# sanonone/kektordb

Measured on AMD Instinct MI355X. Metric: QPS at recall@10>=0.95, 1Mx768 cosine k=10, higher is better.
Workload: dtype f32

## Files before the change

### kektordb_amd/csrc/kdb_search_core.cuh

```cuda
#pragma once
#include "kdb_device.cuh"
#include <math.h>

#ifndef KDB_F32_ROWS2
#define KDB_F32_ROWS2 4
#endif
#ifndef KDB_F32_ROWS6
#define KDB_F32_ROWS6 2
#endif
#ifndef KDB_F32_ROWS
#define KDB_F32_ROWS 3
#endif
#ifndef KDB_F32_DUAL
#define KDB_F32_DUAL 1
#endif
#ifndef KDB_WIDE4_ROWS
#define KDB_WIDE4_ROWS 1
#ifndef KDB_LDS_MERGE
#define KDB_LDS_MERGE 1
#endif
#endif
#ifndef KDB_F16_ROWS
#define KDB_F16_ROWS 2
#endif
#ifdef KDB_SEARCH_TIMERS
#define KDB_T(x) x
#else
#define KDB_T(x)
#endif
namespace kdbcore {

struct WaveLds {
    float *q;
    float *beam_d;
    uint32_t *beam_id;
    uint32_t *nb_id;
    float *nb_d;
    uint32_t *marks;
    uint32_t beam_cap;
    float *nr_d;
    uint32_t *nr_id;
    uint32_t nr_cap;
    uint32_t *nb_lo;
    uint32_t *beam_lo;
    uint32_t *nr_lo;
    uint32_t *ctl;
    float *ins_d;
    uint32_t *ins_id;
    uint32_t ins_cap = 0;
    float qn_up = INFINITY;
};
enum { KDB_W_MB_SEQ = 0,
       KDB_W_MB_ARG = 1,
       KDB_W_LEVEL = 2,
       KDB_W_NEXT2 = 3,
       KDB_W_ROWS_SEQ = 4,
       KDB_W_ROWS_N = 5,
       KDB_W_DONE = 6,
       KDB_W_QNORM = 7,
       KDB_W_ALLOW_LO = 8, KDB_W_ALLOW_HI = 9 };
enum { KDB_W_VISIT = 0u, KDB_W_BEGIN = 1u, KDB_W_EXIT = 2u };
constexpr uint32_t KDB_W_N_SKIP = 0xfffffffdu;
constexpr uint32_t KDB_W_N_EXIT = 0xffffffffu;

__device__ __forceinline__ uint32_t uni(uint32_t x) { return (uint32_t)__builtin_amdgcn_readfirstlane((int)x); }
__device__ __forceinline__ float unif(float x) {
    return __builtin_bit_cast(float, __builtin_amdgcn_readfirstlane(__builtin_bit_cast(int, x)));
}
__device__ __forceinline__ float readlane_f(float x, uint32_t l) {
    return __builtin_bit_cast(float, __builtin_amdgcn_readlane(__builtin_bit_cast(int, x), (int)l));
}
__device__ __forceinline__ uint32_t readlane_u(uint32_t x, uint32_t l) {
    return (uint32_t)__builtin_amdgcn_readlane((int)x, (int)l);
}
__device__ __forceinline__ uint32_t shr1_u(uint32_t x) {
    return (uint32_t)__builtin_amdgcn_update_dpp((int)x, (int)x, 0x138, 0xf, 0xf, false);
}
__device__ __forceinline__ float shr1_f(float x) { return __builtin_bit_cast(float, shr1_u(__builtin_bit_cast(uint32_t, x))); }
__device__ __forceinline__ uint32_t shl1_u(uint32_t x) {
    return (uint32_t)__builtin_amdgcn_update_dpp((int)x, (int)x, 0x130, 0xf, 0xf, false);
}
__device__ __forceinline__ float shl1_f(float x) { return __builtin_bit_cast(float, shl1_u(__builtin_bit_cast(uint32_t, x))); }

__device__ __forceinline__ void wave_lds_fence() {
    __builtin_amdgcn_fence(__ATOMIC_ACQ_REL, "wavefront");
    __builtin_amdgcn_wave_barrier();
}

__device__ __forceinline__ float kdb_sane_key(float key) { return key != key ? INFINITY : key; }

__device__ __forceinline__ uint32_t lds_u32_or(const uint32_t *p, uint32_t i, uint32_t n, uint32_t other) {
    const uint32_t x = p[i];
    return i < n ? x : other;
}
__device__ __forceinline__ float lds_f32_or(const float *p, uint32_t i, uint32_t n, float other) {
    const float x = p[i];
    return i < n ? x : other;
}

__device__ __forceinline__ float kdb_query_norm_up(const float *q, uint32_t ld) {
    double sq = 0.0;
    for (uint32_t i = (uint32_t)kdb_lane(); i < ld; i += 64u) {
        const double y = (double)q[i];
        sq += y * y;
    }
#pragma unroll
    for (int o = 32; o >= 1; o >>= 1) sq += __shfl_xor(sq, o, 64);
    const double nrm = sqrt(sq) * (1.0 + 0x1p-20);
    float f = (float)nrm;
    if ((double)f < nrm) f = __uint_as_float(__float_as_uint(f) + 1u);
    return unif(nrm <= 0x1p20 ? f : INFINITY);
}
__device__ __forceinline__ float kdb_perm_f(uint32_t a, uint32_t b, uint32_t sel) { return __uint_as_float(__builtin_amdgcn_perm(a, b, sel)); }
__device__ __forceinline__ float4 kdb_plane_piece(uint32_t wh, uint32_t wh2, uint32_t wl, uint32_t wl2) {
    return make_float4(kdb_perm_f(wh, wl, 0x05040100u), kdb_perm_f(wh, wl, 0x07060302u), kdb_perm_f(wh2, wl2, 0x05040100u), kdb_perm_f(wh2, wl2, 0x07060302u));
}
__device__ __forceinline__ float4 kdb_plane_piece_hi(uint32_t wh, uint32_t wh2) {
    return make_float4(kdb_perm_f(wh, wh, 0x05040c0cu), kdb_perm_f(wh, wh, 0x07060c0cu), kdb_perm_f(wh2, wh2, 0x05040c0cu), kdb_perm_f(wh2, wh2, 0x07060c0cu));
}
template <int NCH, int RR, bool HI>
__device__ __forceinline__ void kdb_planes_partial(const uint4 (&h)[RR][NCH / 2], const uint4 (&l)[RR][NCH / 2], const float4 (&yq)[NCH], float (&p)[RR]) {
    float a[RR][4];
#pragma unroll
    for (int r = 0; r < RR; r++) a[r][0] = a[r][1] = a[r][2] = a[r][3] = 0.f;
#pragma unroll
    for (int i = 0; i < NCH; i++) {
        const float4 y = yq[i];
#pragma unroll
        for (int r = 0; r < RR; r++) {
            const uint4 wh = h[r][i >> 1], wl = l[r][i >> 1];
            const float4 x = HI ? ((i & 1) ? kdb_plane_piece_hi(wh.z, wh.w) : kdb_plane_piece_hi(wh.x, wh.y))
                                : ((i & 1) ? kdb_plane_piece(wh.z, wh.w, wl.z, wl.w) : kdb_plane_piece(wh.x, wh.y, wl.x, wl.y));
            a[r][0] = __builtin_fmaf(y.x, x.x, a[r][0]);
            a[r][1] = __builtin_fmaf(y.y, x.y, a[r][1]);
            a[r][2] = __builtin_fmaf(y.z, x.z, a[r][2]);
            a[r][3] = __builtin_fmaf(y.w, x.w, a[r][3]);
        }
        __builtin_amdgcn_sched_barrier(0);
    }
#pragma unroll
    for (int r = 0; r < RR; r++) p[r] = (a[r][0] + a[r][1]) + (a[r][2] + a[r][3]);
}
template <int NCH, int RR>
__device__ __forceinline__ void kdb_planes_trip(const KdbView &v, const WaveLds &s, uint32_t base, uint32_t n, int g, int t, bool full, float neg_worst) {
    constexpr int NJ = NCH / 2;
    uint32_t rr[RR];
    size_t off[RR];
    uint4 h[RR][NJ], l[RR][NJ];
    float er[RR];
#pragma unroll
    for (int r = 0; r < RR; r++) {
        rr[r] = base + 4u * (uint32_t)r + (uint32_t)g;
        const uint32_t id = lds_u32_or(s.nb_id, rr[r], n, 0u);
        off[r] = (size_t)id * v.ld;
        const uint4 *hp = reinterpret_cast<const uint4 *>(v.walk_hi + off[r]);
#pragma unroll
        for (int j = 0; j < NJ; j++) h[r][j] = hp[t + 16 * j];
        er[r] = full ? v.walk_err[id] : 0.f;
    }
    float4 yq[NCH];
#pragma unroll
    for (int i = 0; i < NCH; i++) yq[i] = reinterpret_cast<const float4 *>(s.q)[t + 16 * i];
    bool surv[RR];
    if (full) {
        float ph[RR];
        kdb_planes_partial<NCH, RR, true>(h, h, yq, ph);
        bool any = false;
#pragma unroll
        for (int r = 0; r < RR; r++) {
            const float bound = __builtin_fmaf(s.qn_up, er[r], kdb_reduce16(ph[r])) + 0x1p-100f;
            surv[r] = rr[r] < n && !(bound <= neg_worst && bound >= -3.0e38f);
            any = any || surv[r];
        }
        if (__ballot(any) == 0ull) {
#pragma unroll
            for (int r = 0; r < RR; r++)
                if (rr[r] < n && t == 0) s.nb_d[rr[r]] = INFINITY;
            return;
        }
    } else {
#pragma unroll
        for (int r = 0; r < RR; r++) surv[r] = true;
    }
#pragma unroll
    for (int r = 0; r < RR; r++) {
        const uint4 *lp = reinterpret_cast<const uint4 *>(v.walk_lo + (surv[r] ? off[r] : (size_t)0));
#pragma unroll
        for (int j = 0; j < NJ; j++) l[r][j] = lp[t + 16 * j];
    }
    float p[RR];
    kdb_planes_partial<NCH, RR, false>(h, l, yq, p);
#pragma unroll
    for (int r = 0; r < RR; r++) {
        const float key = kdb_key_from_raw<KDB_PREC_F32, KDB_METRIC_COSINE>(kdb_reduce16(p[r]));
        if (rr[r] < n && t == 0) s.nb_d[rr[r]] = surv[r] ? kdb_sane_key(key) : INFINITY;
    }
}

template <int PREC, int METRIC, int NCH = 0, int RMAX = 0, int PL = 0>
__device__ __forceinline__ void compute_dists(const KdbView &v, const WaveLds &s, uint32_t n, float qnorm, bool full = false, float worst = INFINITY) {
    const int lane = kdb_lane();
    const int g = lane >> 4, t = lane & 15;
    if constexpr (PL != 0) {
        static_assert(PREC == KDB_PREC_F32 && METRIC == KDB_METRIC_COSINE && NCH > 0 && NCH <= 12 && NCH % 2 == 0 && RMAX == 0, "walk planes: float32 cosine, ld == 64 * NCH");
        constexpr int R = 2;
        const float neg_worst = unif(-worst);
        full = uni(full ? 1u : 0u) != 0u;
        for (uint32_t base = 0; base < n;) {
            const uint32_t left = n - base;
            if (left > 4u * (R - 1) || R == 1) {
                kdb_planes_trip<NCH, R>(v, s, base, n, g, t, full, neg_worst);
                base += 4u * R;
            } else if (left > 4u) {
                kdb_planes_trip<NCH, 2>(v, s, base, n, g, t, full, neg_worst);
                base += 8u;
            } else {
                kdb_planes_trip<NCH, 1>(v, s, base, n, g, t, full, neg_worst);
                base += 4u;
            }
        }
        wave_lds_fence();
        return;
    }
    if constexpr (PREC == KDB_PREC_F32 && NCH > 0 && NCH <= 16 && KDB_F32_DUAL) {
        constexpr int R0 = NCH <= 2 ? KDB_F32_ROWS2 : NCH <= 6 ? KDB_F32_ROWS6 : NCH <= 12 ? KDB_F32_ROWS : 2;
        constexpr int R = (RMAX > 0 && R0 > RMAX) ? RMAX : R0;
        for (uint32_t base = 0; base < n;) {
            const uint32_t left = n - base;
            if (left > 4u * (R - 1) || R == 1) {
                const float *rows[R];
                uint32_t rr[R];
#pragma unroll
                for (int r = 0; r < R; r++) {
                    rr[r] = base + 4u * (uint32_t)r + (uint32_t)g;
                    const uint32_t id = lds_u32_or(s.nb_id, rr[r], n, 0u);
                    rows[r] = reinterpret_cast<const float *>(v.rows) + (size_t)id * v.ld;
                }
                float p[R];
                kdb_row_partialR_f32<METRIC, NCH, R>(rows, s.q, t, p, v.ld >> 2);
#pragma unroll
                for (int r = 0; r < R; r++) {
                    const float key = kdb_key_from_raw<PREC, METRIC>(kdb_reduce16(p[r]));
                    if (rr[r] < n && t == 0) s.nb_d[rr[r]] = kdb_sane_key(key);
                }
                base += 4u * R;
            } else if (left > 4u) {
                const uint32_t r0 = base + (uint32_t)g, r1 = r0 + 4u;
                const uint32_t id0 = s.nb_id[r0], id1 = lds_u32_or(s.nb_id, r1, n, 0u);
                float p0, p1;
                kdb_row_partial2_f32<METRIC, NCH>(reinterpret_cast<const float *>(v.rows) + (size_t)id0 * v.ld,
                                                  reinterpret_cast<const float *>(v.rows) + (size_t)id1 * v.ld, s.q, t, p0, p1, v.ld >> 2);
                const float k0 = kdb_key_from_raw<PREC, METRIC>(kdb_reduce16(p0));
                const float k1 = kdb_key_from_raw<PREC, METRIC>(kdb_reduce16(p1));
                if (t == 0) s.nb_d[r0] = kdb_sane_key(k0);
                if (r1 < n && t == 0) s.nb_d[r1] = kdb_sane_key(k1);
                base += 8u;
            } else {
                const uint32_t r0 = base + (uint32_t)g;
                const uint32_t id0 = lds_u32_or(s.nb_id, r0, n, 0u);
                const float p = kdb_row_partial_f32<METRIC, NCH>(reinterpret_cast<const float *>(v.rows) + (size_t)id0 * v.ld, s.q, v.ld, t);
                const float k0 = kdb_key_from_raw<PREC, METRIC>(kdb_reduce16(p));
                if (r0 < n && t == 0) s.nb_d[r0] = kdb_sane_key(k0);
                base += 4u;
            }
        }
        wave_lds_fence();
        return;
    }
    if constexpr (PREC == KDB_PREC_F16 && NCH > 0 && NCH % 2 == 0 && NCH <= 24) {
        constexpr int R = (RMAX > 0 && KDB_F16_ROWS > RMAX) ? RMAX : KDB_F16_ROWS;
// ... 894 lines not shown
        }
        count--;
        wave_lds_fence();
    }
    __device__ __forceinline__ void push(float dd, uint32_t dlo, uint32_t idv, float worst, uint32_t worst_lo, bool full) {
        if (count == cap) {
            if (full) {
                const uint32_t lane = (uint32_t)kdb_lane();
                uint32_t w = 0;
                for (uint32_t base = 0; base < count; base += 64) {
                    const uint32_t i = base + lane;
                    float e = 0.f;
                    uint32_t x = 0, el = 0;
                    bool keep = false;
                    if (i < count) {
                        e = d[i];
                        x = id[i];
                        if (WK) el = l[i];
                        keep = !key_lt<WK>(worst, worst_lo, e, el);
                    }
                    const unsigned long long m = __ballot(keep);
                    wave_lds_fence();
                    if (keep) {
                        d[w + kdb_mbcnt(m)] = e;
                        id[w + kdb_mbcnt(m)] = x;
                        if (WK) l[w + kdb_mbcnt(m)] = el;
                    }
                    w += (uint32_t)__builtin_popcountll(m);
                    wave_lds_fence();
                }
                count = w;
            }
            if (count == cap) {
                dropped++;
                if (cap == 0) return;
                float md;
                uint32_t ml, mid;
                const uint32_t mp = extreme<true>(md, ml, mid);
                if (!(key_lt<WK>(dd, dlo, md, ml) || (key_eq<WK>(dd, dlo, md, ml) && idv < mid))) return;
                remove(mp);
            }
        }
        if (kdb_lane() == 0) {
            d[count] = dd;
            id[count] = idv;
            if (WK) l[count] = dlo;
        }
        count++;
        wave_lds_fence();
    }
};
using NrList = NrListT<false>;

struct QCtr {
    uint32_t n_dist, n_hops, n_dropped;
#ifdef KDB_SEARCH_TIMERS
    uint32_t n_ins;
    unsigned long long t_adj, t_dist, t_ins, t_pop, t_vis, t_upper, t_wait, t_pred;
#endif
};

struct EpKnown {
    bool known = false;
    float key = 0.f;
    uint32_t lo = 0u;
};

template <class BeamT, class NrT>
__device__ __forceinline__ void insert_candidates(const KdbView &v, const WaveLds &s, BeamT &b, NrT &nr, uint32_t ef, unsigned long long pass,
                                                  float my_d, uint32_t my_lo, uint32_t my_id, bool my_nr, QCtr &ctr) {
    constexpr bool WK = BeamT::kWide;
    const int lane = kdb_lane();
    if constexpr (BeamT::kSlots >= 1 && !WK) {
        constexpr int S = BeamT::kSlots;
        const uint32_t npass = (uint32_t)__builtin_popcountll(pass);
        if (npass >= 2u && !v.has_deleted && (S == 1 || s.ins_cap >= ef)) {
            const uint32_t m = b.count;
            const bool in_pass = ((pass >> lane) & 1ull) != 0ull;
            bool in_beam[S];
            uint32_t shift[S];
#pragma unroll
            for (int q = 0; q < S; q++) {
                in_beam[q] = 64u * q + (uint32_t)lane < m;
                shift[q] = 0u;
            }
            uint32_t place = 0u;
            bool tie = false;
            for (unsigned long long rest = pass; rest;) {
                const uint32_t j = (uint32_t)__builtin_ctzll(rest);
                rest &= rest - 1ull;
                const float cd = readlane_f(my_d, j);
                uint32_t below = 0u;
#pragma unroll
                for (int q = 0; q < S; q++) {
                    if (64u * q >= m) continue;
                    shift[q] += (in_beam[q] && cd < b.d[q]) ? 1u : 0u;
                    below += (uint32_t)__builtin_popcountll(__ballot(in_beam[q] && b.d[q] < cd));
                    tie = tie || (in_beam[q] && b.d[q] == cd);
                }
                tie = tie || (in_pass && (uint32_t)lane != j && cd == my_d);
                place += (in_pass && cd < my_d) ? 1u : 0u;
                if ((uint32_t)lane == j) place += below;
            }
            if (__ballot(tie) == 0ull) {
                const uint32_t total = m + npass;
                const uint32_t ncount = total < ef ? total : ef;
                const bool c_keep = in_pass && place < ef;
                wave_lds_fence();
#pragma unroll
                for (int q = 0; q < S; q++) {
                    const uint32_t b_to = 64u * q + (uint32_t)lane + shift[q];
                    if (in_beam[q] && b_to < ef) {
                        s.ins_d[b_to] = b.d[q];
// ... 231 lines not shown
    vis.begin_layer(level > 0);
    float ep_key = epk.key;
    uint32_t ep_lo = epk.lo;
    if (!epk.known) {
        if (lane == 0) s.nb_id[0] = ep;
        wave_lds_fence();
        compute_dists<PREC, METRIC, NCH, 0, PL>(v, s, 1, qnorm);
        ep_key = unif(s.nb_d[0]);
        ep_lo = WK ? uni(s.nb_lo[0]) : 0u;
    }
    ctr.n_dist++;
    {
        (void)vis.test_and_set(ep, lane == 0);
        bool no_result = ((v.deleted[ep >> 5] >> (ep & 31)) & 1u) != 0;
        if (allow && !((allow[ep >> 5] >> (ep & 31)) & 1u)) no_result = true;
        if (no_result) {
            nr.push(ep_key, ep_lo, ep, INFINITY, 0u, false);
        } else {
            b.insert(ep_key, ep_lo, ep);
            b.n_res++;
            b.trim(ef);
        }
    }
    const uint32_t deg = level == 0 ? v.deg0 : v.deg_up;
    KDB_T(const unsigned long long tq_layer = __builtin_readcyclecounter();)
    for (;;) {
        KDB_T(const unsigned long long tq_a = __builtin_readcyclecounter();)
        uint32_t cur;
        if (!pop_candidate(b, nr, ef, cur)) break;
        if (cur - 1u >= v.count) continue;
        const uint32_t *adj = v.adj0 + (size_t)cur * v.deg0;
        if (level > 0) {
            const int lv = (int)v.levels[cur];
            const uint32_t upi = v.up_idx[cur];
            if (lv < level) continue;
            adj = v.adj_up + ((size_t)upi + (size_t)(level - 1)) * v.deg_up;
        }
        ctr.n_hops++;
        KDB_T(const unsigned long long tq0 = __builtin_readcyclecounter(); if (level == 0) ctr.t_pop += tq0 - tq_a;)
        const uint32_t nbx = adj[(uint32_t)lane < deg ? (uint32_t)lane : deg - 1u];
        const uint32_t nb = (uint32_t)lane < deg ? nbx : 0u;
        KDB_T(asm volatile("s_waitcnt vmcnt(0) lgkmcnt(0)" ::: "memory"); const unsigned long long tq_v = __builtin_readcyclecounter();)
        bool fresh = vis.test_and_set(nb, nb != 0u && nb <= v.count);
        if (fresh && allow) fresh = ((allow[nb >> 5] >> (nb & 31)) & 1u) != 0;
        const unsigned long long m = __ballot(fresh);
        const uint32_t n = (uint32_t)__builtin_popcountll(m);
        KDB_T(if (level == 0) { ctr.t_adj += tq_v - tq0; ctr.t_vis += __builtin_readcyclecounter() - tq_v; })
        if (n == 0) continue;
        if (fresh) s.nb_id[kdb_mbcnt(m)] = nb;
        wave_lds_fence();
        const uint32_t my_id = lds_u32_or(s.nb_id, (uint32_t)lane, n, 0u);
        const uint32_t delw = ((uint32_t)lane < n && v.has_deleted) ? v.deleted[my_id >> 5] : 0u;
        KDB_T(const unsigned long long tq1 = __builtin_readcyclecounter();)
        compute_dists<PREC, METRIC, NCH, 0, PL>(v, s, n, qnorm, !(b.n_res < ef), b.worst);
        ctr.n_dist += n;
        const bool my_nr = ((delw >> (my_id & 31)) & 1u) != 0;
        const float my_d = lds_f32_or(s.nb_d, (uint32_t)lane, n, INFINITY);
        const uint32_t my_lo = (WK && (uint32_t)lane < n) ? s.nb_lo[lane] : 0u;
        const unsigned long long pass = __ballot((uint32_t)lane < n && (b.n_res < ef || key_lt<WK>(my_d, my_lo, b.worst, b.worst_lo)));
        kdb_tiny_dot_rule<PREC, METRIC>(b, pass, my_d);
        KDB_T(const unsigned long long tq2 = __builtin_readcyclecounter(); if (level == 0) ctr.t_dist += tq2 - tq1;)
        insert_candidates(v, s, b, nr, ef, pass, my_d, my_lo, my_id, my_nr, ctr);
        KDB_T(if (level == 0) ctr.t_ins += __builtin_readcyclecounter() - tq2;)
    }
    KDB_T(if (level > 0) ctr.t_upper += __builtin_readcyclecounter() - tq_layer;)
    ctr.n_dropped += nr.dropped;
    vis.end_layer();
}

template <int PREC, int METRIC, int NCH, class BeamT, int WIDE>
__device__ void search_layer_wide(const KdbView &v, const WaveLds &s, BeamT &b, WideCtx &wc, uint32_t ep, int level, uint32_t ef,
                                  const uint32_t *allow, QCtr &ctr, EpKnown epk = EpKnown()) {
    const int lane = kdb_lane();
    b.reset(ef);
    constexpr bool WK = BeamT::kWide;
    NrListT<WK> nr;
    nr.bind(s);
    if (lane == 0) s.ctl[KDB_W_NEXT2] = 0u;
    if (lane == 0) s.ctl[KDB_W_LEVEL] = (uint32_t)level | (epk.known ? 0x200u : 0x100u);
    wide_request<WIDE>(s, wc, KDB_W_BEGIN, ep);
    if (!epk.known) (void)wide_wait(s, wc);
    const float ep_key = epk.known ? epk.key : unif(s.nb_d[0]);
    const uint32_t ep_lo = epk.known ? epk.lo : (WK ? uni(s.nb_lo[0]) : 0u);
    ctr.n_dist++;
    {
        bool no_result = ((v.deleted[ep >> 5] >> (ep & 31)) & 1u) != 0;
        if (allow && !((allow[ep >> 5] >> (ep & 31)) & 1u)) no_result = true;
        if (no_result) {
            nr.push(ep_key, ep_lo, ep, INFINITY, 0u, false);
        } else {
            b.insert(ep_key, ep_lo, ep);
            b.n_res++;
            b.trim(ef);
        }
    }
    bool asked = epk.known;
    KDB_T(const unsigned long long tq_layer = __builtin_readcyclecounter();)
    for (;;) {
        KDB_T(const unsigned long long tq_a = __builtin_readcyclecounter();)
        uint32_t cur;
        if (!pop_candidate(b, nr, ef, cur)) break;
        if (!asked) wide_request<WIDE>(s, wc, KDB_W_VISIT, cur);
        asked = false;
        {
            const uint32_t h = b.first_pending();
            if (lane == 0) wide_store(s.ctl + KDB_W_NEXT2, h);
        }
// ... 72 lines not shown
```

### kektordb_amd/csrc/probe.hip

```cpp
#include "kdb_internal.h"

namespace {

__device__ __forceinline__ uint32_t mix32(uint32_t x) {
    x ^= x >> 16;
    x *= 0x7feb352du;
    x ^= x >> 15;
    x *= 0x846ca68bu;
    x ^= x >> 16;
    return x;
}

template <int R, int MINW>
__global__ void __launch_bounds__(64, MINW)
gather_probe_kernel(const unsigned char *__restrict__ rows, uint32_t row_bytes, uint32_t count, uint32_t trips, uint32_t seed, uint32_t *sink) {
    const uint32_t lane = threadIdx.x, g = lane >> 4, t = lane & 15u;
    const uint32_t chunks = row_bytes >> 8;
    uint4 acc = make_uint4(0, 0, 0, 0);
    for (uint32_t trip = 0; trip < trips; trip++) {
        const unsigned char *p[R];
#pragma unroll
        for (int r = 0; r < R; r++) {
            const uint32_t id = 1u + mix32(seed ^ (blockIdx.x * 0x9e3779b9u) ^ ((trip * (uint32_t)R + (uint32_t)r) * 4u + g) * 0x85ebca6bu) % count;
            p[r] = rows + (size_t)id * row_bytes + t * 16u;
// ... 26 lines not shown
    for (size_t i = (size_t)blockIdx.x * 256u * 4u + threadIdx.x; i < n16; i += stride) {
        uint4 v[4];
#pragma unroll
        for (int u = 0; u < 4; u++) v[u] = i + (size_t)u * 256u < n16 ? src[i + (size_t)u * 256u] : make_uint4(0, 0, 0, 0);
#pragma unroll
        for (int u = 0; u < 4; u++) {
            acc.x ^= v[u].x;
            acc.y += v[u].y;
            acc.z ^= v[u].z;
            acc.w += v[u].w;
        }
    }
    if ((acc.x ^ acc.y ^ acc.z ^ acc.w) == 0x5a5a5a5au) sink[blockIdx.x] = acc.x;
}

template <int R, int MINW>
int run_gather(const unsigned char *rows, uint32_t row_bytes, uint32_t count, uint64_t n_reads, int n_cu, uint32_t *d_sink, hipStream_t s, float *best_ms,
               uint64_t *reads_done) {
    int occ = 0;
    if (hipOccupancyMaxActiveBlocksPerMultiprocessor(&occ, gather_probe_kernel<R, MINW>, 64, 0) != hipSuccess || occ < 1) occ = 1;
    const uint32_t grid = (uint32_t)n_cu * (uint32_t)occ;
    uint32_t trips = (uint32_t)(n_reads / ((uint64_t)grid * 4u * R));
    if (trips < 1) trips = 1;
    hipEvent_t e0, e1;
    KDB_HIP(hipEventCreate(&e0));
    KDB_HIP(hipEventCreate(&e1));
    float best = 1e30f;
    for (int it = 0; it < 3; it++) {
        KDB_HIP(hipEventRecord(e0, s));
        hipLaunchKernelGGL((gather_probe_kernel<R, MINW>), dim3(grid), dim3(64), 0, s, rows, row_bytes, count, trips, 0x1234u + (uint32_t)it, d_sink);
        KDB_HIP(hipEventRecord(e1, s));
        KDB_HIP(hipEventSynchronize(e1));
        float ms = 0.f;
        KDB_HIP(hipEventElapsedTime(&ms, e0, e1));
        if (ms < best) best = ms;
    }
    (void)hipEventDestroy(e0);
    (void)hipEventDestroy(e1);
    const uint64_t done = (uint64_t)grid * trips * 4u * R;
    const double rate = (double)done / best;
    if (*best_ms <= 0.f || rate > (double)*reads_done / *best_ms) {
        *best_ms = best;
        *reads_done = done;
    }
    return KDB_OK;
}

}

extern "C" int kdb_probe_gather(kdb_index *idx, int which, uint64_t n_reads, float *ms, uint64_t *bytes) {
    if (!idx || !ms || !bytes) return KDB_ERR_INVALID;
    std::lock_guard<std::mutex> lk(idx->mu);
    KDB_HIP(hipSetDevice(idx->device));
    const unsigned char *rows = reinterpret_cast<const unsigned char *>(which ? (const void *)idx->d_rows16 : (const void *)idx->d_rows);
    const uint32_t row_bytes = which ? idx->ld16 * 2u : idx->ld * (uint32_t)idx->elem;
    if (!rows || idx->count == 0 || (row_bytes & 255u)) {
        kdb_set_error("probe_gather: no such row array, no rows, or rows that are not whole 256-byte pieces");
        return KDB_ERR_UNSUPPORTED;
    }
    uint32_t *d_sink = nullptr;
    KDB_HIP(hipMalloc(&d_sink, (size_t)idx->n_cu * 64 * 4));
    float best = 0.f;
    uint64_t reads = 0;
    hipStream_t s = idx->stream;
    int rc = run_gather<2, 4>(rows, row_bytes, idx->count, n_reads, idx->n_cu, d_sink, s, &best, &reads);
    if (!rc) rc = run_gather<3, 2>(rows, row_bytes, idx->count, n_reads, idx->n_cu, d_sink, s, &best, &reads);
    if (!rc) rc = run_gather<4, 2>(rows, row_bytes, idx->count, n_reads, idx->n_cu, d_sink, s, &best, &reads);
    if (!rc) rc = run_gather<2, 2>(rows, row_bytes, idx->count, n_reads, idx->n_cu, d_sink, s, &best, &reads);
    (void)hipFree(d_sink);
    if (rc) return rc;
    *ms = best;
    *bytes = reads * row_bytes;
    return KDB_OK;
}

extern "C" int kdb_probe_stream(kdb_index *idx, int which, float *ms, uint64_t *bytes) {
    if (!idx || !ms || !bytes) return KDB_ERR_INVALID;
    std::lock_guard<std::mutex> lk(idx->mu);
    KDB_HIP(hipSetDevice(idx->device));
    const void *rows = which ? (const void *)idx->d_rows16 : (const void *)idx->d_rows;
    const size_t total = ((size_t)idx->count + 1) * (which ? idx->ld16 * 2u : idx->ld * idx->elem);
    if (!rows || idx->count == 0) {
        kdb_set_error("probe_stream: no such row array or no rows");
        return KDB_ERR_UNSUPPORTED;
    }
    uint32_t *d_sink = nullptr;
    const uint32_t grid = (uint32_t)idx->n_cu * 8u;
    KDB_HIP(hipMalloc(&d_sink, (size_t)grid * 4));
    hipEvent_t e0, e1;
    KDB_HIP(hipEventCreate(&e0));
    KDB_HIP(hipEventCreate(&e1));
    float best = 1e30f;
    for (int it = 0; it < 3; it++) {
        KDB_HIP(hipEventRecord(e0, idx->stream));
        hipLaunchKernelGGL(stream_probe_kernel, dim3(grid), dim3(256), 0, idx->stream, reinterpret_cast<const uint4 *>(rows), total / 16, d_sink);
        KDB_HIP(hipEventRecord(e1, idx->stream));
        KDB_HIP(hipEventSynchronize(e1));
        float t = 0.f;
        KDB_HIP(hipEventElapsedTime(&t, e0, e1));
        if (t < best) best = t;
    }
    (void)hipEventDestroy(e0);
    (void)hipEventDestroy(e1);
    (void)hipFree(d_sink);
    *ms = best;
    *bytes = total / 16 * 16;
    return KDB_OK;
}
// ... 21 lines not shown
```

### kektordb_amd/csrc/search_kernel.cuh

```cuda
#pragma once
#include "kdb_search_core.cuh"
#include <map>
#include <tuple>
#include <mutex>
#include <stdio.h>
#include <stdlib.h>

bool kdb_heap_overlap_begin(const kdb_index *idx, hipStream_t s);
void kdb_heap_overlap_launched(const kdb_index *idx, hipStream_t s, hipEvent_t ev);

#define KDB_LAUNCH_SEARCH_PARAMS                                                                                                    \
    kdb_index *idx, const KdbView &v, const void *d_q, const float *d_qnorm, uint32_t raw, uint32_t B, uint32_t k, uint32_t ef,        \
        const uint32_t *d_allow, KdbMultiAllow ma, uint32_t entry, uint32_t *d_out_ids, float *d_out_dist, uint32_t *d_out_count,      \
        uint32_t *d_tr_ndist, uint32_t *d_tr_nhops, hipStream_t s
#define KDB_LAUNCH_SEARCH_ARGS idx, v, d_q, d_qnorm, raw, B, k, ef, d_allow, ma, entry, d_out_ids, d_out_dist, d_out_count, d_tr_ndist, d_tr_nhops, s

namespace {
using namespace kdbcore;

template <int BS, bool WK> struct BeamSel { using type = RegBeam<BS, WK>; };
template <bool WK> struct BeamSel<0, WK> { using type = LdsBeamT<WK>; };
template <int VIS> struct VisSel { using type = VisBitset; };
template <> struct VisSel<1> { using type = VisHash; };

template <int PREC>
__device__ __forceinline__ size_t q_lds_bytes(uint32_t ld) {
    return PREC == KDB_PREC_I8 ? ((size_t)ld + 15) / 16 * 16 : (size_t)ld * 4;
}

#ifndef KDB_F16_MINW
#define KDB_F16_MINW 3
#endif
#ifndef KDB_F32_MINW6
#define KDB_F32_MINW6 4
#endif
#ifndef KDB_F32_MINW
#define KDB_F32_MINW 2
#endif
#ifndef KDB_WIDE4_MINW
#define KDB_WIDE4_MINW 4
#endif
#ifndef KDB_WIDE4_MINW_LONG
#define KDB_WIDE4_MINW_LONG 2
#endif
#ifndef KDB_SEARCH_MINW
#define KDB_SEARCH_MINW 4
#endif
#ifndef KDB_GENERIC_MINW
#define KDB_GENERIC_MINW 3
#endif
template <int PREC, int NCH, int WIDE>
constexpr int kdb_search_minw() {
    if (WIDE == 4 && KDB_WIDE4_MINW) return NCH > 16 ? KDB_WIDE4_MINW_LONG : NCH == 0 ? (KDB_WIDE4_MINW > 3 ? 3 : KDB_WIDE4_MINW) : KDB_WIDE4_MINW;
    if (WIDE == 2 && NCH > 16) return 2;
    if (PREC == KDB_PREC_I8) return 4;
    if (PREC == KDB_PREC_F16) return NCH > 16 ? 2 : KDB_F16_MINW;
    return NCH > 12 ? 2 : NCH > 6 ? KDB_F32_MINW : NCH > 4 ? KDB_F32_MINW6 : NCH == 0 ? KDB_GENERIC_MINW : KDB_SEARCH_MINW;
}
template <int PREC, int METRIC, int NCH>
constexpr bool kdb_planes_kernel() { return PREC == KDB_PREC_F32 && METRIC == KDB_METRIC_COSINE && NCH == 12; }
template <int PREC, int METRIC, int NCH, int BS, int VIS, int WIDE = 1, int PL = 0>
__global__ void __launch_bounds__(64 * WIDE, (kdb_search_minw<PREC, NCH, WIDE>()))
hnsw_search_kernel(KdbView v, const void *__restrict__ queries, const float *__restrict__ qnorms, uint32_t raw, uint32_t B,
                   uint32_t k, uint32_t ef, const uint32_t *__restrict__ allow, KdbMultiAllow ma, uint32_t entry,
                   uint32_t beam_cap, uint32_t nr_cap, uint32_t vis_size, uint32_t *visited_pool, uint32_t *work,
                   unsigned long long *gctr, uint32_t *out_ids, float *out_dist, uint32_t *out_count,
                   uint32_t *tr_ndist, uint32_t *tr_nhops, uint32_t *tie_list ,
                   unsigned char *tie_stash ) {
    extern __shared__ __attribute__((aligned(16))) unsigned char smem[];
    WaveLds s;
    size_t off = 0;
    s.q = reinterpret_cast<float *>(smem + off);
    off += q_lds_bytes<PREC>(v.ld);
    s.beam_d = reinterpret_cast<float *>(smem + off);
    if (BS == 0) off += (size_t)beam_cap * 4;
    s.beam_id = reinterpret_cast<uint32_t *>(smem + off);
    if (BS == 0) off += (size_t)beam_cap * 4;
    s.beam_lo = reinterpret_cast<uint32_t *>(smem + off);
    if (BS == 0 && PREC == KDB_PREC_I8) off += (size_t)beam_cap * 4;
    s.nb_id = reinterpret_cast<uint32_t *>(smem + off);
    off += 64 * 4;
    s.nb_d = reinterpret_cast<float *>(smem + off);
    off += 64 * 4;
    s.nb_lo = PREC == KDB_PREC_I8 ? reinterpret_cast<uint32_t *>(smem + off) : nullptr;
    if (PREC == KDB_PREC_I8) off += 64 * 4;
    s.ctl = reinterpret_cast<uint32_t *>(smem + off);
    if (WIDE > 1) off += 64;
    s.ins_d = s.nb_d;
    s.ins_id = s.nb_id;
    s.ins_cap = 64u;
    if (WIDE > 1 || BS >= 2) {
        constexpr uint32_t ins_n = 64u * (BS >= 2 ? (uint32_t)BS : 1u);
        s.ins_d = reinterpret_cast<float *>(smem + off);
        off += ins_n * 4;
        s.ins_id = reinterpret_cast<uint32_t *>(smem + off);
        off += ins_n * 4;
        s.ins_cap = ins_n;
    }
    s.nr_d = reinterpret_cast<float *>(smem + off);
    off += (size_t)nr_cap * 4;
    s.nr_id = reinterpret_cast<uint32_t *>(smem + off);
    off += (size_t)nr_cap * 4;
    s.nr_lo = reinterpret_cast<uint32_t *>(smem + off);
    if (PREC == KDB_PREC_I8) off += (size_t)nr_cap * 4;
    s.nr_cap = nr_cap;
    s.marks = reinterpret_cast<uint32_t *>(smem + off);
    s.beam_cap = beam_cap;

    const int lane = kdb_lane();
    typename VisSel<VIS>::type vis;
    if constexpr (VIS == 1) {
        vis.tab = s.marks;
        vis.full_size = vis_size;
        vis.bs.bits = visited_pool + (size_t)blockIdx.x * v.vis_words;
        vis.bs.words = v.vis_words;
// ... 61 lines not shown
            layer(ep, l, 1u);
            const int best = b.first_result();
            if (best < 0) failed = true;
            else {
                float bd_;
                uint32_t bl_, bf_;
                b.get((uint32_t)best, bd_, bl_, bf_);
                ep = bf_ & KDB_ID_MASK;
                epk.known = true;
                epk.key = bd_;
                epk.lo = bl_;
            }
        }
        uint32_t nout = 0;
        if (!failed) layer(ep, 0, ef);
        const bool requeue = b.tied && (raw & 16u) && tie_list != nullptr;
        const bool aside = requeue && (raw & 32u);
        const KdbTieStash st{tie_stash, B, k};
        uint32_t *const o_ids = aside ? st.ids(qi) : out_ids + (size_t)qi * k;
        float *const o_dist = aside ? st.dist(qi) : out_dist + (size_t)qi * k;
        double *const o_dist64 = aside ? st.dist64(qi) : reinterpret_cast<double *>(out_dist) + (size_t)qi * k;
        if (!failed) {
            nout = b.write_results(k, o_ids, o_dist, PREC == KDB_PREC_F32 && METRIC == KDB_METRIC_COSINE,
                                   (PREC == KDB_PREC_I8 && (raw & 4u)) ? o_dist64 : nullptr);
        }
        for (uint32_t p = nout + (uint32_t)lane; p < k; p += 64) {
            o_ids[p] = 0u;
            if (PREC == KDB_PREC_I8 && (raw & 4u)) o_dist64[p] = (double)INFINITY;
            else o_dist[p] = INFINITY;
        }
        if (lane == 0) {
            if (aside) {
                uint32_t *const m = st.meta(qi);
                m[0] = nout | ((raw & 8u) ? 0x80000000u : 0u);
                m[1] = ctr.n_dist;
                m[2] = ctr.n_hops;
            } else {
                out_count[qi] = nout | ((b.tied && (raw & 8u)) ? 0x80000000u : 0u);
                if (tr_ndist) tr_ndist[qi] = ctr.n_dist;
                if (tr_nhops) tr_nhops[qi] = ctr.n_hops;
                if (requeue) tie_list[4u + atomicAdd(tie_list, 1u)] = qi;
            }
        }
        if (aside) {
            __builtin_amdgcn_fence(__ATOMIC_RELEASE, "agent");
            if (lane == 0) {
                const uint32_t old = atomicExch(&tie_list[4u + atomicAdd(tie_list, 1u)], qi);
                asm volatile("" ::"v"(old) : "memory");
            }
        }
        if (ma.done_flags && !requeue) kdb_publish_done(ma.done_flags + qi, ma.done_gen);
        tot_tied += b.tied;
        if (requeue) ctr.n_dist = ctr.n_hops = ctr.n_dropped = 0u;
        KDB_T(if (lane == 0 && qi < 64u) printf("q %u waves %d: hops %u dist %u inserts %u | cycles: total %llu upper-layers %llu | level 0: pop %llu list %llu visited %llu rows %llu predict+post %llu predict+post+insert %llu wait-for-wave-1 %llu | wave 1: visit %llu cycles, hint hits %u\n", qi, WIDE, ctr.n_hops, ctr.n_dist, ctr.n_ins, __builtin_readcyclecounter() - tq_start, ctr.t_upper, ctr.t_pop, ctr.t_adj, ctr.t_vis, ctr.t_dist, ctr.t_pred, ctr.t_ins, ctr.t_wait, WIDE > 1 ? *reinterpret_cast<unsigned long long *>(s.ctl + 12) : 0ull, WIDE > 1 ? s.ctl[14] : 0u);)
        tot_dist += ctr.n_dist;
        tot_hops += ctr.n_hops;
        tot_dropped += ctr.n_dropped;
        wave_lds_fence();
    }
    if constexpr (WIDE > 1) wide_request<WIDE>(s, wc, KDB_W_EXIT, 0u);
    if (lane == 0) {
        unsigned long long *acc = reinterpret_cast<unsigned long long *>(work) - 2;
        const unsigned long long r0 = atomicAdd(&acc[0], tot_dist);
        const unsigned long long r1 = atomicAdd(&acc[1], tot_hops);
        const unsigned long long r3 = tot_dropped ? atomicAdd(&acc[3], tot_dropped) : 0ull;
        const unsigned long long r4 = tot_tied ? atomicAdd(&acc[4], tot_tied) : 0ull;
        asm volatile("" ::"v"(r0), "v"(r1), "v"(r3), "v"(r4) : "memory");
        if (atomicAdd(work + 1, 1u) == gridDim.x - 1u) {
            if (tie_list && (raw & 32u)) {
                const unsigned long long o0 = atomicExch(&gctr[0], atomicExch(&acc[0], 0ull));
                const unsigned long long o1 = atomicExch(&gctr[1], atomicExch(&acc[1], 0ull));
                const unsigned long long o3 = atomicExch(&gctr[3], atomicExch(&acc[3], 0ull));
                const unsigned long long o2 = atomicExch(&gctr[2], atomicExch(&acc[4], 0ull));
                const unsigned long long ow = atomicExch(&acc[2], 0ull);
                asm volatile("" ::"v"(o0), "v"(o1), "v"(o3), "v"(o2), "v"(ow) : "memory");
                atomicExch(&tie_list[2], 1u);
            } else {
                gctr[0] = atomicExch(&acc[0], 0ull);
                gctr[1] = atomicExch(&acc[1], 0ull);
                gctr[3] = atomicExch(&acc[3], 0ull);
                gctr[2] = atomicExch(&acc[4], 0ull);
                atomicExch(&acc[2], 0ull);
            }
        }
    }
}

template <typename K>
int occupancy_blocks(K kern, int threads, size_t lds) {
    static std::mutex mu;
    static std::map<std::tuple<const void *, size_t, int, int>, int> cache;
    int dev = 0;
    (void)hipGetDevice(&dev);
    const std::tuple<const void *, size_t, int, int> key(reinterpret_cast<const void *>(kern), lds, dev, threads);
    std::lock_guard<std::mutex> lk(mu);
    auto it = cache.find(key);
    if (it != cache.end()) return it->second;
    int nb = 0;
    if (hipOccupancyMaxActiveBlocksPerMultiprocessor(&nb, kern, threads, lds) != hipSuccess || nb < 1) nb = 1;
    cache[key] = nb;
    return nb;
}

template <int PREC, int METRIC, int NCH, int BS>
static int launch_search_bs(kdb_index *idx, const KdbView &v, const void *d_q, const float *d_qnorm, uint32_t raw, uint32_t B,
                            uint32_t k, uint32_t ef, const uint32_t *d_allow, KdbMultiAllow ma, uint32_t entry, uint32_t *d_out_ids,
                            float *d_out_dist, uint32_t *d_out_count, uint32_t *d_tr_ndist, uint32_t *d_tr_nhops,
// ... 209 lines not shown
```

### kektordb_amd/index.py

```python
from __future__ import annotations

import ctypes as C
from dataclasses import dataclass
from typing import List, Optional, Sequence

import numpy as np

from . import _lib
from ._lib import KdbError, check

L2, COSINE = 0, 1
F32, F16, I8 = 0, 1, 2
SEARCH_NEEDS_REFINE = 1
SEARCH_PREPARED = 2
SEARCH_DIST_F64 = 8
SEARCH_TIE_FLAG = 16
SEARCH_HEAP_ORDER = 32
VACUUM_ELECT_TOP_LEVEL = 1
COUNT_TIED = 0x80000000
COUNT_MASK = 0x7fffffff

_ELEM = {F32: np.float32, F16: np.uint16, I8: np.int8}


# ... 286 lines not shown

    def flat_scan_batch(self, queries, k: int, allow_bits=None, dist64: bool = False):
        self._live()
        q = np.ascontiguousarray(queries, dtype=np.float32)
        B = q.shape[0]
        ids = np.zeros((B, k), dtype=np.uint32)
        dist = np.full((B, k), np.inf, dtype=np.float64 if dist64 else np.float32)
        cnt = np.zeros(B, dtype=np.uint32)
        ab = None if allow_bits is None else np.ascontiguousarray(allow_bits, dtype=np.uint64)
        check(self.L.kdb_flat_scan_batch(self.h, _ptr(q), B, k, _ptr(ab), self._flags() | (SEARCH_DIST_F64 if dist64 else 0), _ptr(ids), _ptr(dist),
                                         _ptr(cnt)), "kdb_flat_scan_batch")
        return ids, dist, cnt

    def flat_scan_batch_dev(self, d_queries, k, d_out_ids, d_out_dist, d_out_count, d_allow=None, stream=None, dist64=False):
        self._live()
        _ready(stream)
        B = d_queries.shape[0]
        check(self.L.kdb_flat_scan_batch_dev(self.h, _tptr(d_queries), B, k, _tptr(d_allow), self._flags() | (SEARCH_DIST_F64 if dist64 else 0),
                                             _tptr(d_out_ids), _tptr(d_out_dist), _tptr(d_out_count),
                                             C.c_void_p(stream) if stream else None), "kdb_flat_scan_batch_dev")

    def distance_batch(self, queries, ids, prepared=False):
        self._live()
        q = np.ascontiguousarray(queries, dtype=np.float32)
        ii = np.ascontiguousarray(ids, dtype=np.uint32)
        B, Cn = ii.shape
        out = np.zeros((B, Cn), dtype=np.float32)
        check(self.L.kdb_distance_batch(self.h, _ptr(q), B, _ptr(ii), Cn, self._flags(prepared), _ptr(out)),
              "kdb_distance_batch")
        return out

    def distance_batch_dev(self, d_queries, d_ids, d_out, stream=None, prepared=False):
        _ready(stream)
        B, Cn = d_ids.shape
        check(self.L.kdb_distance_batch_dev(self.h, _tptr(d_queries), B, _tptr(d_ids), Cn, self._flags(prepared),
                                            _tptr(d_out), C.c_void_p(stream) if stream else None),
              "kdb_distance_batch_dev")

    def counters(self):
        c = _lib.Counters()
        check(self.L.kdb_get_counters(self.h, C.byref(c)), "get_counters")
        return {"n_dist": int(c.n_dist), "n_hops": int(c.n_hops), "bytes": int(c.bytes),
                "kernel_ms": float(c.last_kernel_ms), "n_dropped": int(c.n_dropped), "n_tied": int(c.n_tied)}

    def launch_stats(self, last_n: int):
        arr = (_lib.Counters * last_n)()
        check(self.L.kdb_get_launch_stats(self.h, last_n, arr), "get_launch_stats")
        return [{"n_dist": int(c.n_dist), "n_hops": int(c.n_hops), "bytes": int(c.bytes),
                 "kernel_ms": float(c.last_kernel_ms), "n_dropped": int(c.n_dropped), "n_tied": int(c.n_tied)} for c in arr]

    def sync(self):
        check(self.L.kdb_index_sync(self.h), "sync")

    def probe_gather(self, n_reads: int = 4_000_000, shadow: bool = False):
        ms, nbytes = C.c_float(), C.c_uint64()
        check(self.L.kdb_probe_gather(self.h, 1 if shadow else 0, n_reads, C.byref(ms), C.byref(nbytes)), "kdb_probe_gather")
        return nbytes.value / (ms.value * 1e-3) / 1e9

    def poison_lds(self, pattern: int = 0):
        check(self.L.kdb_probe_poison_lds(self.h, int(pattern) & 0xffffffff), "kdb_probe_poison_lds")

    def probe_stream(self, shadow: bool = False):
        ms, nbytes = C.c_float(), C.c_uint64()
        check(self.L.kdb_probe_stream(self.h, 1 if shadow else 0, C.byref(ms), C.byref(nbytes)), "kdb_probe_stream")
        return nbytes.value / (ms.value * 1e-3) / 1e9

    def merge_topk_dev(self, G, B, k, d_in_ids, d_in_dist, d_in_count, d_id_base, d_out_ids, d_out_dist, d_out_count,
                       stream=None):
        check(self.L.kdb_merge_topk_dev(self.h, G, B, k, _tptr(d_in_ids), _tptr(d_in_dist), _tptr(d_in_count),
                                        _tptr(d_id_base), _tptr(d_out_ids), _tptr(d_out_dist), _tptr(d_out_count),
                                        C.c_void_p(stream) if stream else None), "kdb_merge_topk_dev")

    def search_batch_multi_dev(self, d_queries, k: int, ef: int, d_allow_lists, d_allow_of_query, d_out_ids, d_out_dist,
                               d_out_count, stream=None, tie_flag=False, heap_order=False):
        self._live()
        _ready(stream)
        B = int(d_queries.shape[0])
        G, words = int(d_allow_lists.shape[0]), int(d_allow_lists.shape[1])
        check(self.L.kdb_search_batch_multi_dev(self.h, _tptr(d_queries), B, k, ef, _tptr(d_allow_lists), G, words,
                                                _tptr(d_allow_of_query), self._flags(False) | (SEARCH_TIE_FLAG if tie_flag else 0)
                                                | (SEARCH_HEAP_ORDER if heap_order else 0), _tptr(d_out_ids), _tptr(d_out_dist),
                                                _tptr(d_out_count), C.c_void_p(stream) if stream else None),
              "kdb_search_batch_multi_dev")

    def flat_scan_groups_dev(self, d_queries, k: int, group_offsets, d_allow_lists, d_out_ids, d_out_dist, d_out_count,
                             max_total_allowed: int = 0, stream=None):
        self._live()
        _ready(stream)
        off = np.ascontiguousarray(group_offsets, dtype=np.uint32)
        B = int(d_queries.shape[0])
        G, words = int(d_allow_lists.shape[0]), int(d_allow_lists.shape[1])
        assert off.size == G + 1
        check(self.L.kdb_flat_scan_groups_dev(self.h, _tptr(d_queries), B, k, G, _ptr(off), _tptr(d_allow_lists), words,
                                              int(max_total_allowed), self._flags(False), _tptr(d_out_ids), _tptr(d_out_dist),
                                              _tptr(d_out_count), C.c_void_p(stream) if stream else None),
              "kdb_flat_scan_groups_dev")

    def merge_topk_packed_dev(self, G, B, k, d_packed, stride_words, d_id_base, d_out_ids, d_out_dist, d_out_count,
                              stream=None):
        check(self.L.kdb_merge_topk_packed_dev(self.h, G, B, k, _tptr(d_packed), stride_words, _tptr(d_id_base),
                                               _tptr(d_out_ids), _tptr(d_out_dist), _tptr(d_out_count),
                                               C.c_void_p(stream) if stream else None), "kdb_merge_topk_packed_dev")

    def merge_topk_packed_f64_dev(self, G, B, k, d_packed, stride_words, d_id_base, d_out_ids, d_out_dist, d_out_count, stream=None):
        check(self.L.kdb_merge_topk_packed_f64_dev(self.h, G, B, k, _tptr(d_packed), stride_words, _tptr(d_id_base),
                                                   _tptr(d_out_ids), _tptr(d_out_dist), _tptr(d_out_count),
                                                   C.c_void_p(stream) if stream else None), "kdb_merge_topk_packed_f64_dev")

    def score(self, raw: float) -> float:
# ... 55 lines not shown
```

Measured before the change: 4.412 million.

## Cut register use in walk-plane distance loop and raise planes kernel occupancy bound

```diff
diff --git a/kektordb_amd/csrc/kdb_search_core.cuh b/kektordb_amd/csrc/kdb_search_core.cuh
--- a/kektordb_amd/csrc/kdb_search_core.cuh
+++ b/kektordb_amd/csrc/kdb_search_core.cuh
@@ -24,11 +24,21 @@
 #define KDB_F16_ROWS 2
 #endif
 #ifdef KDB_SEARCH_TIMERS
-#define KDB_T(x) x
+#define KDB_T(...) __VA_ARGS__
 #else
-#define KDB_T(x)
+#define KDB_T(...)
 #endif
 namespace kdbcore {
+
+struct QCtr {
+    uint32_t n_dist, n_hops, n_dropped;
+#ifdef KDB_SEARCH_TIMERS
+    uint32_t n_ins;
+    unsigned long long t_adj, t_dist, t_ins, t_pop, t_vis, t_upper, t_wait, t_pred;
+    unsigned long long t_hi_wait, t_hi_math, t_lo_wait, t_lo_math, t_notfull;
+    uint32_t n_eval_hops, n_two_trips, n_trips, n_trips_lo;
+#endif
+};
 
 struct WaveLds {
     float *q;
@@ -119,18 +129,22 @@
     return make_float4(kdb_perm_f(wh, wh, 0x05040c0cu), kdb_perm_f(wh, wh, 0x07060c0cu), kdb_perm_f(wh2, wh2, 0x05040c0cu), kdb_perm_f(wh2, wh2, 0x07060c0cu));
 }
 template <int NCH, int RR, bool HI>
-__device__ __forceinline__ void kdb_planes_partial(const uint4 (&h)[RR][NCH / 2], const uint4 (&l)[RR][NCH / 2], const float4 (&yq)[NCH], float (&p)[RR]) {
+__device__ __forceinline__ void kdb_planes_partial(const uint4 (&h)[RR][NCH / 2], const uint4 (&l)[RR][NCH / 2], const float4 *yq, float (&p)[RR]) {
     float a[RR][4];
 #pragma unroll
     for (int r = 0; r < RR; r++) a[r][0] = a[r][1] = a[r][2] = a[r][3] = 0.f;
+    float4 yn = yq[0];
 #pragma unroll
     for (int i = 0; i < NCH; i++) {
-        const float4 y = yq[i];
+        const float4 y = yn;
+        if (i + 1 < NCH) yn = yq[16 * (i + 1)];
 #pragma unroll
         for (int r = 0; r < RR; r++) {
             const uint4 wh = h[r][i >> 1], wl = l[r][i >> 1];
-            const float4 x = HI ? ((i & 1) ? kdb_plane_piece_hi(wh.z, wh.w) : kdb_plane_piece_hi(wh.x, wh.y))
-                                : ((i & 1) ? kdb_plane_piece(wh.z, wh.w, wl.z, wl.w) : kdb_plane_piece(wh.x, wh.y, wl.x, wl.y));
+            uint32_t h0 = (i & 1) ? wh.z : wh.x, h1 = (i & 1) ? wh.w : wh.y, l0 = (i & 1) ? wl.z : wl.x, l1 = (i & 1) ? wl.w : wl.y;
+            if (HI) asm volatile("" : "+v"(h0), "+v"(h1), "+v"(a[r][0]), "+v"(a[r][1]), "+v"(a[r][2]), "+v"(a[r][3]));
+            else asm volatile("" : "+v"(h0), "+v"(h1), "+v"(l0), "+v"(l1), "+v"(a[r][0]), "+v"(a[r][1]), "+v"(a[r][2]), "+v"(a[r][3]));
+            const float4 x = HI ? kdb_plane_piece_hi(h0, h1) : kdb_plane_piece(h0, h1, l0, l1);
             a[r][0] = __builtin_fmaf(y.x, x.x, a[r][0]);
             a[r][1] = __builtin_fmaf(y.y, x.y, a[r][1]);
             a[r][2] = __builtin_fmaf(y.z, x.z, a[r][2]);
@@ -142,7 +156,7 @@
     for (int r = 0; r < RR; r++) p[r] = (a[r][0] + a[r][1]) + (a[r][2] + a[r][3]);
 }
 template <int NCH, int RR>
-__device__ __forceinline__ void kdb_planes_trip(const KdbView &v, const WaveLds &s, uint32_t base, uint32_t n, int g, int t, bool full, float neg_worst) {
+__device__ __forceinline__ void kdb_planes_trip(const KdbView &v, const WaveLds &s, uint32_t base, uint32_t n, int g, int t, bool full, float neg_worst KDB_T(, QCtr *tc)) {
     constexpr int NJ = NCH / 2;
     uint32_t rr[RR];
     size_t off[RR];
@@ -158,12 +172,12 @@
         for (int j = 0; j < NJ; j++) h[r][j] = hp[t + 16 * j];
         er[r] = full ? v.walk_err[id] : 0.f;
     }
-    float4 yq[NCH];
-#pragma unroll
-    for (int i = 0; i < NCH; i++) yq[i] = reinterpret_cast<const float4 *>(s.q)[t + 16 * i];
+    const float4 *yq = reinterpret_cast<const float4 *>(s.q) + t;
     bool surv[RR];
+    KDB_T(unsigned long long tp0 = __builtin_readcyclecounter(); if (tc) tc->n_trips++;)
     if (full) {
         float ph[RR];
+        KDB_T(asm volatile("s_waitcnt vmcnt(0) lgkmcnt(0)" ::: "memory"); if (tc) { const unsigned long long c = __builtin_readcyclecounter(); tc->t_hi_wait += c - tp0; tp0 = c; })
         kdb_planes_partial<NCH, RR, true>(h, h, yq, ph);
         bool any = false;
 #pragma unroll
@@ -172,6 +186,7 @@
             surv[r] = rr[r] < n && !(bound <= neg_worst && bound >= -3.0e38f);
             any = any || surv[r];
         }
+        KDB_T(if (tc) { const unsigned long long c = __builtin_readcyclecounter(); tc->t_hi_math += c - tp0; tp0 = c; })
         if (__ballot(any) == 0ull) {
 #pragma unroll
             for (int r = 0; r < RR; r++)
@@ -189,16 +204,18 @@
         for (int j = 0; j < NJ; j++) l[r][j] = lp[t + 16 * j];
     }
     float p[RR];
+    KDB_T(if (full) { asm volatile("s_waitcnt vmcnt(0) lgkmcnt(0)" ::: "memory"); if (tc) { const unsigned long long c = __builtin_readcyclecounter(); tc->t_lo_wait += c - tp0; tp0 = c; tc->n_trips_lo++; } })
     kdb_planes_partial<NCH, RR, false>(h, l, yq, p);
 #pragma unroll
     for (int r = 0; r < RR; r++) {
         const float key = kdb_key_from_raw<KDB_PREC_F32, KDB_METRIC_COSINE>(kdb_reduce16(p[r]));
         if (rr[r] < n && t == 0) s.nb_d[rr[r]] = surv[r] ? kdb_sane_key(key) : INFINITY;
     }
+    KDB_T(if (tc) { const unsigned long long c = __builtin_readcyclecounter(); if (full) tc->t_lo_math += c - tp0; else tc->t_notfull += c - tp0; })
 }
 
 template <int PREC, int METRIC, int NCH = 0, int RMAX = 0, int PL = 0>
-__device__ __forceinline__ void compute_dists(const KdbView &v, const WaveLds &s, uint32_t n, float qnorm, bool full = false, float worst = INFINITY) {
+__device__ __forceinline__ void compute_dists(const KdbView &v, const WaveLds &s, uint32_t n, float qnorm, bool full = false, float worst = INFINITY KDB_T(, QCtr *tc = nullptr)) {
     const int lane = kdb_lane();
     const int g = lane >> 4, t = lane & 15;
     if constexpr (PL != 0) {
@@ -209,13 +226,13 @@
         for (uint32_t base = 0; base < n;) {
             const uint32_t left = n - base;
             if (left > 4u * (R - 1) || R == 1) {
-                kdb_planes_trip<NCH, R>(v, s, base, n, g, t, full, neg_worst);
+                kdb_planes_trip<NCH, R>(v, s, base, n, g, t, full, neg_worst KDB_T(, tc));
                 base += 4u * R;
             } else if (left > 4u) {
-                kdb_planes_trip<NCH, 2>(v, s, base, n, g, t, full, neg_worst);
+                kdb_planes_trip<NCH, 2>(v, s, base, n, g, t, full, neg_worst KDB_T(, tc));
                 base += 8u;
             } else {
-                kdb_planes_trip<NCH, 1>(v, s, base, n, g, t, full, neg_worst);
+                kdb_planes_trip<NCH, 1>(v, s, base, n, g, t, full, neg_worst KDB_T(, tc));
                 base += 4u;
             }
         }
@@ -1216,13 +1233,6 @@
 };
 using NrList = NrListT<false>;
 
-struct QCtr {
-    uint32_t n_dist, n_hops, n_dropped;
-#ifdef KDB_SEARCH_TIMERS
-    uint32_t n_ins;
-    unsigned long long t_adj, t_dist, t_ins, t_pop, t_vis, t_upper, t_wait, t_pred;
-#endif
-};
 
 struct EpKnown {
     bool known = false;
@@ -1560,7 +1570,8 @@
         const uint32_t my_id = lds_u32_or(s.nb_id, (uint32_t)lane, n, 0u);
         const uint32_t delw = ((uint32_t)lane < n && v.has_deleted) ? v.deleted[my_id >> 5] : 0u;
         KDB_T(const unsigned long long tq1 = __builtin_readcyclecounter();)
-        compute_dists<PREC, METRIC, NCH, 0, PL>(v, s, n, qnorm, !(b.n_res < ef), b.worst);
+        KDB_T(if (level == 0) { ctr.n_eval_hops++; if (n > 8u) ctr.n_two_trips++; })
+        compute_dists<PREC, METRIC, NCH, 0, PL>(v, s, n, qnorm, !(b.n_res < ef), b.worst KDB_T(, level == 0 ? &ctr : nullptr));
         ctr.n_dist += n;
         const bool my_nr = ((delw >> (my_id & 31)) & 1u) != 0;
         const float my_d = lds_f32_or(s.nb_d, (uint32_t)lane, n, INFINITY);
diff --git a/kektordb_amd/csrc/probe.hip b/kektordb_amd/csrc/probe.hip
--- a/kektordb_amd/csrc/probe.hip
+++ b/kektordb_amd/csrc/probe.hip
@@ -102,8 +102,12 @@
     if (!idx || !ms || !bytes) return KDB_ERR_INVALID;
     std::lock_guard<std::mutex> lk(idx->mu);
     KDB_HIP(hipSetDevice(idx->device));
-    const unsigned char *rows = reinterpret_cast<const unsigned char *>(which ? (const void *)idx->d_rows16 : (const void *)idx->d_rows);
-    const uint32_t row_bytes = which ? idx->ld16 * 2u : idx->ld * (uint32_t)idx->elem;
+    if (which < 0 || which > 2) {
+        kdb_set_error("probe_gather: which is 0 (rows), 1 (half-precision copy) or 2 (high walk plane)");
+        return KDB_ERR_INVALID;
+    }
+    const unsigned char *rows = reinterpret_cast<const unsigned char *>(which == 2 ? (const void *)idx->d_walk_hi : which ? (const void *)idx->d_rows16 : (const void *)idx->d_rows);
+    const uint32_t row_bytes = which == 2 ? idx->ld * 2u : which ? idx->ld16 * 2u : idx->ld * (uint32_t)idx->elem;
     if (!rows || idx->count == 0 || (row_bytes & 255u)) {
         kdb_set_error("probe_gather: no such row array, no rows, or rows that are not whole 256-byte pieces");
         return KDB_ERR_UNSUPPORTED;
diff --git a/kektordb_amd/csrc/search_kernel.cuh b/kektordb_amd/csrc/search_kernel.cuh
--- a/kektordb_amd/csrc/search_kernel.cuh
+++ b/kektordb_amd/csrc/search_kernel.cuh
@@ -37,6 +37,9 @@
 #ifndef KDB_F32_MINW
 #define KDB_F32_MINW 2
 #endif
+#ifndef KDB_PLANES_MINW
+#define KDB_PLANES_MINW 3
+#endif
 #ifndef KDB_WIDE4_MINW
 #define KDB_WIDE4_MINW 4
 #endif
@@ -49,8 +52,9 @@
 #ifndef KDB_GENERIC_MINW
 #define KDB_GENERIC_MINW 3
 #endif
-template <int PREC, int NCH, int WIDE>
+template <int PREC, int NCH, int WIDE, int PL = 0, int BS = 0>
 constexpr int kdb_search_minw() {
+    if (PL != 0 && BS == 1 && WIDE == 1) return KDB_PLANES_MINW;
     if (WIDE == 4 && KDB_WIDE4_MINW) return NCH > 16 ? KDB_WIDE4_MINW_LONG : NCH == 0 ? (KDB_WIDE4_MINW > 3 ? 3 : KDB_WIDE4_MINW) : KDB_WIDE4_MINW;
     if (WIDE == 2 && NCH > 16) return 2;
     if (PREC == KDB_PREC_I8) return 4;
@@ -60,7 +64,7 @@
 template <int PREC, int METRIC, int NCH>
 constexpr bool kdb_planes_kernel() { return PREC == KDB_PREC_F32 && METRIC == KDB_METRIC_COSINE && NCH == 12; }
 template <int PREC, int METRIC, int NCH, int BS, int VIS, int WIDE = 1, int PL = 0>
-__global__ void __launch_bounds__(64 * WIDE, (kdb_search_minw<PREC, NCH, WIDE>()))
+__global__ void __launch_bounds__(64 * WIDE, (kdb_search_minw<PREC, NCH, WIDE, PL, BS>()))
 hnsw_search_kernel(KdbView v, const void *__restrict__ queries, const float *__restrict__ qnorms, uint32_t raw, uint32_t B,
                    uint32_t k, uint32_t ef, const uint32_t *__restrict__ allow, KdbMultiAllow ma, uint32_t entry,
                    uint32_t beam_cap, uint32_t nr_cap, uint32_t vis_size, uint32_t *visited_pool, uint32_t *work,
@@ -228,7 +232,7 @@
         if (ma.done_flags && !requeue) kdb_publish_done(ma.done_flags + qi, ma.done_gen);
         tot_tied += b.tied;
         if (requeue) ctr.n_dist = ctr.n_hops = ctr.n_dropped = 0u;
-        KDB_T(if (lane == 0 && qi < 64u) printf("q %u waves %d: hops %u dist %u inserts %u | cycles: total %llu upper-layers %llu | level 0: pop %llu list %llu visited %llu rows %llu predict+post %llu predict+post+insert %llu wait-for-wave-1 %llu | wave 1: visit %llu cycles, hint hits %u\n", qi, WIDE, ctr.n_hops, ctr.n_dist, ctr.n_ins, __builtin_readcyclecounter() - tq_start, ctr.t_upper, ctr.t_pop, ctr.t_adj, ctr.t_vis, ctr.t_dist, ctr.t_pred, ctr.t_ins, ctr.t_wait, WIDE > 1 ? *reinterpret_cast<unsigned long long *>(s.ctl + 12) : 0ull, WIDE > 1 ? s.ctl[14] : 0u);)
+        KDB_T(if (lane == 0 && qi < 64u) printf("q %u waves %d: hops %u dist %u inserts %u | cycles: total %llu upper-layers %llu | level 0: pop %llu list %llu visited %llu rows %llu predict+post %llu predict+post+insert %llu wait-for-wave-1 %llu | wave 1: visit %llu cycles, hint hits %u | planes %d: level-0 hops with new neighbours %u, with more than 8 %u, trips %u, with a low-plane trip %u, cycles high-wait %llu high-math %llu low-wait %llu low-math %llu not-full %llu\n", qi, WIDE, ctr.n_hops, ctr.n_dist, ctr.n_ins, __builtin_readcyclecounter() - tq_start, ctr.t_upper, ctr.t_pop, ctr.t_adj, ctr.t_vis, ctr.t_dist, ctr.t_pred, ctr.t_ins, ctr.t_wait, WIDE > 1 ? *reinterpret_cast<unsigned long long *>(s.ctl + 12) : 0ull, WIDE > 1 ? s.ctl[14] : 0u, PL, ctr.n_eval_hops, ctr.n_two_trips, ctr.n_trips, ctr.n_trips_lo, ctr.t_hi_wait, ctr.t_hi_math, ctr.t_lo_wait, ctr.t_lo_math, ctr.t_notfull);)
         tot_dist += ctr.n_dist;
         tot_hops += ctr.n_hops;
         tot_dropped += ctr.n_dropped;
diff --git a/kektordb_amd/index.py b/kektordb_amd/index.py
--- a/kektordb_amd/index.py
+++ b/kektordb_amd/index.py
@@ -362,9 +362,9 @@
     def sync(self):
         check(self.L.kdb_index_sync(self.h), "sync")
 
-    def probe_gather(self, n_reads: int = 4_000_000, shadow: bool = False):
+    def probe_gather(self, n_reads: int = 4_000_000, shadow: bool = False, walk_hi: bool = False):
         ms, nbytes = C.c_float(), C.c_uint64()
-        check(self.L.kdb_probe_gather(self.h, 1 if shadow else 0, n_reads, C.byref(ms), C.byref(nbytes)), "kdb_probe_gather")
+        check(self.L.kdb_probe_gather(self.h, 2 if walk_hi else 1 if shadow else 0, n_reads, C.byref(ms), C.byref(nbytes)), "kdb_probe_gather")
         return nbytes.value / (ms.value * 1e-3) / 1e9
 
     def poison_lds(self, pattern: int = 0):
```

Measured after the change: 5.127 million, median of 6. 1.16x the previous value.
